# cmavro/GNN-RAG

Measured on AMD Instinct MI355X. Metric: kg_edges_aggregated_per_sec, higher is better.
Workload: dtype f32

## Files before the change

gnn-rag_amd/_lib.py:

```python
from __future__ import annotations

import ctypes as C
import os

PKG = os.path.dirname(os.path.abspath(__file__))
LIB_PATH = os.path.join(PKG, "lib", "libgnnrag_hip.so")

c_i32p = C.POINTER(C.c_int32)
c_f32p = C.POINTER(C.c_float)


class CsrStruct(C.Structure):
    _fields_ = [
        ("B", C.c_int32), ("N", C.c_int32), ("R1", C.c_int32), ("heavy_deg", C.c_int32),
        ("F", C.c_int64),
        ("row_ptr", C.c_void_p * 2), ("edge", C.c_void_p * 2), ("perm", C.c_void_p * 2),
        ("w_gnn", C.c_void_p * 2), ("w_rel", C.c_void_p * 2),
        ("heavy", C.c_void_p * 2), ("chunk_off", C.c_void_p * 2),
        ("n_heavy", C.c_void_p), ("n_chunks", C.c_void_p),
        ("heavy_cap", C.c_int32), ("max_chunks", C.c_int32),
        ("big_cnt", C.c_void_p), ("big_nodes", C.c_void_p),
        ("big_deg", C.c_int32), ("hub_sorted", C.c_int32),
        ("edge_l", C.c_void_p * 2), ("rel_off", C.c_void_p), ("rel_rows", C.c_void_p),
        ("rel_total", C.c_int32), ("rel_max", C.c_int32),
# ... 81 lines not shown
                                            C.c_int32, C.c_int32, _VP]),
    "gnnrag_update_score": (C.c_int, [_VP, _VP, _VP, _VP, _VP, _VP, _VP, _VP, _VP, C.c_int64, C.c_int32,
                                      C.c_int32, C.c_int32, _VP]),
    "gnnrag_dense_form": (C.c_int, [C.c_int32, C.c_int64, C.c_int32, C.c_int32, C.c_int32, C.c_int32, C.c_int64,
                                    C.c_int32, C.c_int32, C.POINTER(DenseFormStruct)]),
    "gnnrag_masked_softmax": (C.c_int, [_VP, _VP, C.c_int32, C.c_int32, _VP]),
    "gnnrag_typelayer": (C.c_int, [C.POINTER(CsrStruct), _VP, C.c_int, _VP, C.c_int32, _VP, C.c_size_t, _VP]),
    "gnnrag_layer_workspace_bytes": (C.c_size_t, [C.POINTER(CsrStruct), C.c_int32, C.c_int32]),
    "gnnrag_stack_workspace_bytes": (C.c_size_t, [C.POINTER(CsrStruct), C.c_int32, C.c_int32, C.c_int32]),
    "gnnrag_rel_transform": (C.c_int, [_VP, _VP, C.c_int64, C.c_int32, C.c_int32, C.POINTER(LayerParams), C.c_int32, _VP,
                                      _VP, _VP]),
    "gnnrag_gemm_tn_workspace_bytes": (C.c_size_t, [C.c_int64, C.c_int32, C.c_int32]),
    "gnnrag_gemm_tn": (C.c_int, [_VP, _VP, C.c_int64, C.c_int32, C.c_int32, _VP, _VP, C.c_size_t, _VP]),
    "gnnrag_rel_planes_bytes": (C.c_size_t, [C.c_int64, C.c_int32, C.c_int32]),
    "gnnrag_relation_tables_planes": (C.c_int, [C.POINTER(CsrStruct), _VP, _VP, _VP, _VP, C.c_int32, C.c_int32, _VP]),
    "gnnrag_reason_layer": (C.c_int, [C.POINTER(CsrStruct)] + [_VP] * 9 + [C.c_int32] + [_VP] * 8 +
                            [_VP, C.c_size_t, C.c_int32, C.c_int32, C.c_int32, C.c_int32, _VP]),
    "gnnrag_reason_stack": (C.c_int, [C.POINTER(CsrStruct), C.c_int32, C.POINTER(LayerParams)] + [_VP] * 5 +
                            [C.c_int32] + [_VP] * 6 + [_VP, C.c_size_t, C.c_int32, C.c_int32, C.c_int32, C.c_int32, _VP]),
    "gnnrag_reason_stack_capture": (C.c_int, [C.POINTER(CsrStruct), C.c_int32, C.POINTER(LayerParams)] + [_VP] * 5 +
                                    [C.c_int32] + [_VP] * 6 + [_VP, C.c_size_t, C.c_int32, C.c_int32, C.c_int32,
                                                               C.c_int32, _VP, C.POINTER(C.c_void_p)]),
    "gnnrag_graph_launch": (C.c_int, [_VP, _VP]),
    "gnnrag_graph_destroy": (C.c_int, [_VP]),
    "gnnrag_frontier_workspace_bytes": (C.c_size_t, [C.POINTER(CsrStruct)]),
    "gnnrag_frontier_supported": (C.c_int, [C.POINTER(CsrStruct), C.c_int32]),
    "gnnrag_frontier_build": (C.c_int, [C.POINTER(CsrStruct), _VP, _VP, C.c_size_t, _VP]),
    "gnnrag_relation_tables_frontier": (C.c_int, [C.POINTER(CsrStruct), _VP, _VP, _VP, _VP, _VP, _VP, C.c_int32,
                                                  C.c_int32, _VP]),
    "gnnrag_aggregate_fused_frontier": (C.c_int, [C.POINTER(CsrStruct), _VP, _VP, _VP, _VP, C.c_int32, _VP]),
# ... 99 lines not shown
```

gnn-rag_amd/csrc/dense_internal.h:

```cpp
#pragma once
#include "gnnrag_common.h"

namespace gnnrag {

int tables_vq_launch_z(const gnnrag_csr* csr, const void* planes, const float* ins, const float* W, float* P, int32_t D,
                       int32_t I, int32_t only_dir, float* zero, int64_t zero_n, hipStream_t stream);

int update_score_fused_rows(const float* h, const float* nbr, const uint8_t* add_flag, const float* W, const float* b,
                            const float* w_s, const float* b_s, const float* mask, float* h_out, float* score,
                            int64_t BN, int32_t D, int32_t I, int32_t math, hipStream_t stream, bool score_zeroed);
int update_b3_launch_f(const float* h, const float* nbr, const uint8_t* add_flag, const float* W, const float* b,
                       const float* w_s, const float* b_s, const float* mask, float* h_out, float* score, int64_t BN,
                       int32_t D, int32_t ldw, hipStream_t stream, bool score_zeroed);

bool update_rows_supported(const float* h, const float* nbr, const float* W, const float* h_out, int64_t BN, int32_t D,
                           int32_t I, int32_t math);
bool update_b3_shape_ok(int64_t BN, int32_t D, int32_t ldw);
int tables_small_launch(const gnnrag_csr* csr, const float* T_fwd, const float* T_inv, const float* ins, const float* W,
                        float* P, int32_t D, int32_t I, hipStream_t stream);

int frontier_build_z(const gnnrag_csr* csr, const float* dist, void* fws, size_t fws_bytes, float* zero_a,
                     int64_t zero_na, float* zero_b, int64_t zero_nb, hipStream_t stream);
const uint8_t* frontier_row_flags(const gnnrag_csr* csr, const void* fws);

int update_score_fused_z(const float* h, const float* nbr, const float* W, const float* b, const float* w_s,
                         const float* b_s, const float* mask, float* h_out, float* score, int64_t BN, int32_t D,
                         int32_t I, int32_t math, hipStream_t stream, bool score_zeroed);

bool rel_transform_accepts(const float* relfeat_fwd, const float* relfeat_inv, int64_t R1, int32_t D, int32_t L,
                           const gnnrag_layer_params* layers, int32_t pos_rows, const float* T_out, const void* planes_out);

}
```

gnn-rag_amd/csrc/rel_transform.hip:

```cpp
#include "gnnrag_common.h"
#include "dense_internal.h"

namespace gnnrag {

constexpr int kRtMaxL = 8;
constexpr int kRtUnroll = 7;

struct RelTArgs {
  const float* A[2];
  const float* W[kRtMaxL];
  const float* b[kRtMaxL];
  const float* add[kRtMaxL][2];
  float* C;
  unsigned short* planes;
  int M, K, N, add_rows;
};

constexpr int kPlaneHalf = 224;
constexpr int kPlaneRow = 2 * kPlaneHalf;

template <int TPW>
__global__ __launch_bounds__(256) void k_rel_transform(RelTArgs g) {
  extern __shared__ __attribute__((aligned(16))) float Wf[];
  const int tid = threadIdx.x, lane = tid & 63, wave = tid >> 6;
  const int fr = lane & 15, fg = lane >> 4;
  const int j = blockIdx.z >> 1, d = blockIdx.z & 1;
  const int colg = blockIdx.y * 64;
  const int K = g.K;
  const int nch = (K + 15) >> 4;
  const f32x4 zero4 = {0.f, 0.f, 0.f, 0.f};
  const bool compute = colg < g.N;
  if (compute) {
    const int total = 64 * nch * 4;
    for (int x = tid; x < total; x += 256) {
// ... 1 lines not shown
      f32x4 v = zero4;
      if (colg + col < g.N && 4 * kq < K) v = *reinterpret_cast<const f32x4*>(g.W[j] + (size_t)(colg + col) * K + 4 * kq);
      const int c = kq >> 2, fgq = kq & 3, a = col & 3, frq = col >> 2;
      *reinterpret_cast<f32x4*>(Wf + ((size_t)((c * 4 + a) * 64 + fgq * 16 + frq)) * 4) = v;
    }
  }
  __syncthreads();
  const int c4 = colg + 4 * fr;
  const bool in_T = c4 < g.N;
  const bool in_pad = !in_T && c4 < kPlaneHalf;
  f32x4 bias = zero4;
  if (in_T && g.b[j]) bias = *reinterpret_cast<const f32x4*>(g.b[j] + c4);
  const float* __restrict__ addp = g.add[j][d];
  float* __restrict__ cp = g.C + ((size_t)(2 * j + d) * g.M) * g.N;
  unsigned short* pp = g.planes ? g.planes + ((size_t)(2 * j + d) * 3 * g.M) * kPlaneRow : nullptr;

#pragma unroll 1
  for (int t = 0; t < TPW; ++t) {
    const int row0 = (blockIdx.x * TPW + t) * 64 + wave * 16;
    if (row0 >= g.M) break;
    f32x4 acc[4][2];
#pragma unroll
    for (int a = 0; a < 4; ++a) acc[a][0] = acc[a][1] = zero4;
    if (compute) {
      const float* __restrict__ ap = g.A[d] + (size_t)min(row0 + fr, g.M - 1) * K;
      for (int c0 = 0; c0 < nch; c0 += kRtUnroll) {
        f32x4 av[kRtUnroll];
#pragma unroll
        for (int u = 0; u < kRtUnroll; ++u)
          av[u] = *reinterpret_cast<const f32x4*>(ap + min(16 * (c0 + u) + 4 * fg, K - 4));
// ... 1 lines not shown
        for (int u = 0; u < kRtUnroll; ++u) {
          const int c = min(c0 + u, nch - 1);
          const bool live = 16 * (c0 + u) + 4 * fg < K;
          const f32x4 x = live ? av[u] : zero4;
          f32x4 wv[4];
#pragma unroll
          for (int a = 0; a < 4; ++a) wv[a] = *reinterpret_cast<const f32x4*>(Wf + ((size_t)((c * 4 + a) * 64 + lane)) * 4);
#pragma unroll
          for (int e = 0; e < 4; ++e)
#pragma unroll
            for (int a = 0; a < 4; ++a)
              acc[a][e & 1] = __builtin_amdgcn_mfma_f32_16x16x4f32(x[e], wv[a][e], acc[a][e & 1], 0, 0, 0);
        }
      }
    }
    if (!in_T && !(pp && in_pad)) continue;
#pragma unroll
    for (int r = 0; r < 4; ++r) {
      const int row = row0 + 4 * fg + r;
      if (row >= g.M) continue;
      f32x4 v = zero4;
      if (in_T) {
#pragma unroll
        for (int a = 0; a < 4; ++a) v[a] = acc[a][0][r] + acc[a][1][r];
        v += bias;
        if (addp && row < g.add_rows) v += *reinterpret_cast<const f32x4*>(addp + (size_t)row * g.N + c4);
        *reinterpret_cast<f32x4*>(cp + (size_t)row * g.N + c4) = v;
      }
      if (pp) {
#pragma unroll
        for (int half = 0; half < 2; ++half) {
          const Split3 sp = split3(__builtin_elementwise_max(half ? -v : v, zero4));
          const size_t e = (size_t)row * kPlaneRow + half * kPlaneHalf + c4;
          *reinterpret_cast<uint2*>(pp + e) = sp.hi;
          *reinterpret_cast<uint2*>(pp + (size_t)g.M * kPlaneRow + e) = sp.mid;
          *reinterpret_cast<uint2*>(pp + (size_t)2 * g.M * kPlaneRow + e) = sp.lo;
        }
      }
    }
  }
}

}

using namespace gnnrag;

extern "C" size_t gnnrag_rel_planes_bytes(int64_t R1, int32_t D, int32_t L) {
  if (R1 <= 0 || D <= 0 || D > kPlaneHalf || L <= 0) return 0;
  return (size_t)L * 2 * 3 * R1 * kPlaneRow * sizeof(unsigned short);
}

bool gnnrag::rel_transform_accepts(const float* relfeat_fwd, const float* relfeat_inv, int64_t R1, int32_t D, int32_t L,
                                   const gnnrag_layer_params* layers, int32_t pos_rows, const float* T_out,
                                   const void* planes_out) {
  if (D <= 0 || (D & 3)) return false;
  if (planes_out && D > kPlaneHalf) return false;
  if (R1 >= ((int64_t)1 << 31) / D) return false;
  uintptr_t align = (uintptr_t)relfeat_fwd | (uintptr_t)relfeat_inv | (uintptr_t)T_out | (uintptr_t)planes_out;
  for (int j = 0; j < L; ++j) {
    align |= (uintptr_t)layers[j].W_rel | (uintptr_t)layers[j].b_rel;
    if (pos_rows > 0) align |= (uintptr_t)layers[j].pos_fwd | (uintptr_t)layers[j].pos_inv;
  }
  if (align & 15) return false;
  return (size_t)64 * ((D + 15) / 16) * 16 * sizeof(float) <= 160 * 1024;
}

extern "C" int gnnrag_rel_transform(const float* relfeat_fwd, const float* relfeat_inv, int64_t R1, int32_t D,
                                    int32_t L, const gnnrag_layer_params* layers, int32_t pos_rows, float* T_out,
                                    void* planes_out, gnnrag_stream_t stream) {
  if (!relfeat_fwd || !relfeat_inv || !layers || !T_out || R1 < 0 || D <= 0 || L <= 0 || pos_rows < 0)
    return GNNRAG_E_BADARG;
  for (int j = 0; j < L; ++j) {
    if (!layers[j].W_rel) return GNNRAG_E_BADARG;
    if ((layers[j].pos_fwd == nullptr) != (layers[j].pos_inv == nullptr)) return GNNRAG_E_BADARG;
  }
  if (!gnnrag::rel_transform_accepts(relfeat_fwd, relfeat_inv, R1, D, L, layers, pos_rows, T_out, planes_out))
    return GNNRAG_E_UNSUPPORTED;
  if (R1 == 0) return 0;
  for (int j0 = 0; j0 < L; j0 += kRtMaxL) {
    const int n = L - j0 < kRtMaxL ? L - j0 : kRtMaxL;
    RelTArgs g;
    memset(&g, 0, sizeof(g));
    g.A[0] = relfeat_fwd;
    g.A[1] = relfeat_inv;
    for (int j = 0; j < n; ++j) {
      const gnnrag_layer_params& p = layers[j0 + j];
      g.W[j] = p.W_rel;
      g.b[j] = p.b_rel;
      g.add[j][0] = pos_rows > 0 ? p.pos_fwd : nullptr;
      g.add[j][1] = pos_rows > 0 ? p.pos_inv : nullptr;
    }
    g.C = T_out + (size_t)j0 * 2 * R1 * D;
    g.planes = planes_out ? (unsigned short*)planes_out + (size_t)j0 * 2 * 3 * R1 * kPlaneRow : nullptr;
    g.M = (int)R1; g.K = D; g.N = D;
    g.add_rows = (int)(pos_rows < R1 ? pos_rows : R1);
    const unsigned gy = (unsigned)(((planes_out ? kPlaneHalf : D) + 63) / 64), gz = (unsigned)(2 * n);
    const size_t lds = (size_t)64 * ((D + 15) / 16) * 16 * sizeof(float);
    static DeviceMask cap1, cap4;
    if (R1 > 2048) {
      if (lds > 64 * 1024) { const int rc = raise_lds_cap(k_rel_transform<4>, cap4); if (rc) return rc; }
      hipLaunchKernelGGL(k_rel_transform<4>, dim3((unsigned)((R1 + 255) / 256), gy, gz), dim3(256), lds,
                         (hipStream_t)stream, g);
    } else {
      if (lds > 64 * 1024) { const int rc = raise_lds_cap(k_rel_transform<1>, cap1); if (rc) return rc; }
      hipLaunchKernelGGL(k_rel_transform<1>, dim3((unsigned)((R1 + 63) / 64), gy, gz), dim3(256), lds,
                         (hipStream_t)stream, g);
    }
    GNNRAG_LAUNCH_CHECK();
  }
  return 0;
}
```

gnn-rag_amd/csrc/softmax_layer.hip:

```cpp
#include "gnnrag_common.h"
#include "dense_internal.h"

namespace gnnrag {

template <int ITEMS>
__global__ __launch_bounds__(1024) void k_masked_softmax(const float* __restrict__ score,
                                                         float* __restrict__ dist, int N) {
  __shared__ float red[16];
  __shared__ float bcast;
  const float* s = score + (size_t)blockIdx.x * N;
  float* o = dist + (size_t)blockIdx.x * N;
  const int lane = threadIdx.x & 63, wave = threadIdx.x >> 6;
  float v[ITEMS > 0 ? ITEMS : 1];

  float m = -INFINITY;
  if constexpr (ITEMS > 0) {
#pragma unroll
    for (int k = 0; k < ITEMS; ++k) {
      const int i = threadIdx.x + k * 1024;
      v[k] = i < N ? s[i] : -INFINITY;
      m = fmaxf(m, v[k]);
    }
  } else {
    for (int i = threadIdx.x; i < N; i += 1024) m = fmaxf(m, s[i]);
// ... 256 lines not shown
      if (!gated) GNNRAG_HIP(hipMemsetAsync(nbr, 0, (size_t)BN * D * sizeof(float), (hipStream_t)stream));
      rc = frontier_build_z(csr, dist, fws, w.fws_bytes, score_out, BN, nbr + (size_t)BN * D, D, (hipStream_t)stream);
      if (rc) return rc;
      rc = gnnrag_relation_tables_frontier(csr, fws, T_fwd, T_inv, ins, W_e2e, P, D, I, stream);
      if (rc) return rc;
      rc = gnnrag_aggregate_fused_frontier(csr, fws, dist, P, nbr, D, stream);
      if (rc) return rc;
      rc = update_score_fused_rows(h, nbr, gated ? frontier_row_flags(csr, fws) : nullptr, W_e2e, b_e2e, w_score, b_score,
                                   mask, h_out, score_out, BN, D, I, math, (hipStream_t)stream, true);
      if (rc) return rc;
      return finish_softmax(csr, w, base, score_out, dist_out, D, only < 0, pairs_for_next, stream);
    }
    rc = GNNRAG_E_UNSUPPORTED;
    bool score_zeroed = false;
    if (planes && math != GNNRAG_MATH_FP32 && csr->rel_total > 0) {
      rc = tables_vq_launch_z(csr, planes, ins, W_e2e, P, D, I, one_dir ? only : -1, score_out, BN, (hipStream_t)stream);
      score_zeroed = rc == 0;
    }
    if (rc == GNNRAG_E_UNSUPPORTED) rc = gnnrag_relation_tables(csr, T_fwd, T_inv, ins, W_e2e, P, D, I, math, stream);
    if (rc) return rc;
    rc = aggregate_fused_dirs(csr, dist, P, nbr, D, one_dir ? 2 - only : 0, base + w.partial, w.partial_bytes,
                              (hipStream_t)stream, pairs_ready && !one_dir);
    if (rc) return rc;
    rc = update_score_fused_z(h, nbr, W_e2e, b_e2e, w_score, b_score, mask, h_out, score_out, BN, D, I, math,
                              (hipStream_t)stream, score_zeroed);
    if (rc) return rc;
    return finish_softmax(csr, w, base, score_out, dist_out, D, only < 0, pairs_for_next, stream);
  } else {
    float* agg = (float*)(base + w.agg);
    rc = gnnrag_aggregate(csr, dist, ins, T_fwd, T_inv, agg, D, I, base + w.partial, w.partial_bytes, stream);
    if (rc) return rc;
    rc = gnnrag_update_score(h, agg, W_e2e, b_e2e, w_score, b_score, mask, h_out, score_out, BN, D, I, math,
                             stream);
    if (rc) return rc;
  }
  return gnnrag_masked_softmax(score_out, dist_out, csr->B, csr->N, stream);
}

static int rel_projections(const gnnrag_csr* csr, int32_t n, const gnnrag_layer_params* layers,
                           const float* relfeat_fwd, const float* relfeat_inv, int32_t pos_rows, float* T,
                           void* planes, bool* planes_written, int32_t D, int32_t math, gnnrag_stream_t stream) {
  *planes_written = false;
  if ((D & 3) == 0) {
    const int rc = gnnrag_rel_transform(relfeat_fwd, relfeat_inv, csr->R1, D, n, layers, pos_rows, T, planes, stream);
    if (rc == 0) *planes_written = planes != nullptr;
    if (rc != GNNRAG_E_UNSUPPORTED) return rc;
  }
  const size_t RD = (size_t)csr->R1 * D;
  for (int j = 0; j < n; ++j) {
    const gnnrag_layer_params& p = layers[j];
    const int rc = gnnrag_linear_pair(relfeat_fwd, relfeat_inv, csr->R1, D, p.W_rel, p.b_rel, p.pos_fwd, p.pos_inv,
                                      p.pos_fwd ? pos_rows : 0, T + 2 * j * RD, T + (2 * j + 1) * RD, D, math, stream);
    if (rc) return rc;
  }
  return 0;
}

extern "C" size_t gnnrag_stack_workspace_bytes(const gnnrag_csr* csr, int32_t L, int32_t D, int32_t I) {
  if (!csr || L <= 0 || D <= 0 || I <= 0) return 0;
// ... 38 lines not shown
  if (!csr || L <= 0 || !layers || !h0 || !dist0 || !ins || !relfeat_fwd || !relfeat_inv || !w_score || !b_score ||
      !mask || !h_out || !score_out || !dist_out || !workspace || D <= 0 || I <= 0)
    return GNNRAG_E_BADARG;
  if (!path_ok(path)) return GNNRAG_E_BADARG;
  for (int j = 0; j < L; ++j)
    if (!layers[j].W_rel || !layers[j].b_rel || !layers[j].W_e2e || !layers[j].b_e2e) return GNNRAG_E_BADARG;
  const LayerWs w = layer_ws(csr, D, I);
  if (workspace_bytes < w.total) return GNNRAG_E_WORKSPACE;
  char* base = (char*)workspace;
  const size_t BN = (size_t)csr->B * csr->N;
  const size_t RD = (size_t)csr->R1 * D;
  const bool upfront = L > 1 && workspace_bytes >= gnnrag_stack_workspace_bytes(csr, L, D, I);
  float* T0 = (float*)(base + w.T_fwd);
  float* Tall = (float*)(base + w.total);
  const bool want_planes = planes_wanted(csr, D, I, path, math);
  const size_t plane_bytes = tables_vq_planes_bytes(csr->R1);
  char* planes_all = base + w.total + align_up((size_t)L * 2 * RD * sizeof(float), 256);
  bool planes_written = false;
  const bool reuse = upfront && (path & GNNRAG_PATH_REUSE_PROJ) != 0;
  path &= ~GNNRAG_PATH_REUSE_PROJ;
  if (reuse) {
    planes_written = want_planes && rel_transform_accepts(relfeat_fwd, relfeat_inv, csr->R1, D, L, layers, pos_rows, Tall,
                                                          planes_all);
  } else if (upfront) {
    const int rc = rel_projections(csr, L, layers, relfeat_fwd, relfeat_inv, pos_rows, Tall,
                                   want_planes ? planes_all : nullptr, &planes_written, D, math, stream);
    if (rc) return rc;
  }
  const float* h = h0;
  const float* dist = dist0;
  bool pairs_ready = false;
// ... 92 lines not shown
```

gnn-rag_amd/csrc/tables_b3.hip:

```cpp
#include "gnnrag_common.h"
#include "dense_internal.h"
#include "b3_tile.h"
#include <type_traits>

namespace gnnrag {

#ifndef GNNRAG_TAB_TPW
#define GNNRAG_TAB_TPW 3
#endif
#ifndef GNNRAG_TAB_MINBLK
#define GNNRAG_TAB_MINBLK 2
#endif
constexpr int kTabTPW = GNNRAG_TAB_TPW;
constexpr int kTabQBytes = 160 * 1024 - 3 * kTabPlaneB - 64;

struct TabArgs {
  const float* T[2];
  const float* ins;
  const float* W;
  float* P;
  const int2* rows;
  int32_t M, D, I, ldw;
  int32_t ct0;
  int32_t npass;
// ... 258 lines not shown
#pragma unroll
  for (int pl = 0; pl < 3; ++pl) {
    const uint4 c = make_uint4(r.p[pl].x | r.n[pl].x, r.p[pl].y | r.n[pl].y, r.p[pl].z | r.n[pl].z, r.p[pl].w | r.n[pl].w);
    o.pl[pl] = __builtin_bit_cast(bf16x8, c);
  }
  const unsigned m[4] = {r.n[0].x | r.n[1].x | r.n[2].x, r.n[0].y | r.n[1].y | r.n[2].y, r.n[0].z | r.n[1].z | r.n[2].z,
                         r.n[0].w | r.n[1].w | r.n[2].w};
  unsigned ix = 0x8888u;
#pragma unroll
  for (int i = 0; i < 4; ++i)
    ix |= (min(m[i] & 0xffffu, 1u) | (min(m[i] >> 16, 1u) << 2)) << (4 * i);
  o.idx = (int)ix;
  return o;
}

template <int CTN>
__device__ __forceinline__ void tables_vq_part(const VqArgs& a, unsigned char* lds, int col0) {
  constexpr int RB = kTabRowB, PL = kTabPlaneB;
  constexpr int NPAIR = (kVqTPW + 1) / 2;
  const int tid = threadIdx.x, lane = tid & 63, wave = tid >> 6;
  const int fr = lane & 15, fg = lane >> 4;
  const int d = a.dir0 + blockIdx.y;
  const int g = blockIdx.x / a.nchunk, ch = blockIdx.x - g * a.nchunk;
  const int D = a.D, I = a.I;
  const int r0 = a.rel_off[g], r1 = a.rel_off[g + 1];
  if (r1 <= r0) return;
  const int ncol = min(CTN * 16, D - col0);
  const f32x4 zero4 = {0.f, 0.f, 0.f, 0.f};
  float* P = a.P + (size_t)d * a.M * D;
  const unsigned char* planes = a.planes + (size_t)d * 3 * a.R1 * kVqRowB;
  const size_t plane_stride = (size_t)a.R1 * kVqRowB;

  const int U = (r1 - r0 + 15) >> 4;
  const int c0 = U * ch / a.nchunk, c1 = U * (ch + 1) / a.nchunk;
  const int wv = __builtin_amdgcn_readfirstlane(wave);
  const int w0 = c0 + (c1 - c0) * wv / 8, w1 = c0 + (c1 - c0) * (wv + 1) / 8;
  const int npass = ((c1 - c0 + 7) / 8 + kVqTPW - 1) / kVqTPW;

  float* qarea = reinterpret_cast<float*>(lds + 3 * PL + 64);
  for (int x = tid * 4; x < I * D; x += 512 * 4)
    *reinterpret_cast<f32x4*>(qarea + x) = *reinterpret_cast<const f32x4*>(a.ins + (size_t)g * I * D + x);

  for (int pass = 0; pass < npass; ++pass) {
    const int tbase = w0 + pass * kVqTPW;
    const int ntile = max(0, min(kVqTPW, w1 - tbase));
    f32x4 acc[kVqTPW][CTN];
#pragma unroll
    for (int j = 0; j < kVqTPW; ++j)
#pragma unroll
      for (int nt = 0; nt < CTN; ++nt) acc[j][nt] = zero4;
    unsigned aoff[kVqTPW];
#pragma unroll
    for (int j = 0; j < kVqTPW; ++j) {
      const int m = min(r0 + (tbase + (j < ntile ? j : 0)) * 16 + fr, r1 - 1);
      aoff[j] = (unsigned)a.rows[m].y * (unsigned)kVqRowB + (unsigned)fg * 16u;
    }
    const unsigned char* const plane_base[3] = {planes, planes + plane_stride, planes + 2 * plane_stride};

    for (int s = 0; s < 3; ++s) {
      __syncthreads();
      const int nblk = s < 2 ? 3 : 1;
      vq_stage<CTN, GNNRAG_VQ_UN>(a, lds, qarea, col0, ncol, d, 3 * s, nblk);
      __syncthreads();
      for (int kb = 0; kb < nblk; ++kb) {
        const int blk = 3 * s + kb;
        const unsigned char* wb = lds + fr * RB + kb * 64 + fg * 16;
#pragma unroll
        for (int p = 0; p < NPAIR; ++p) {
          const int j0 = 2 * p, j1 = 2 * p + 1 < kVqTPW ? 2 * p + 1 : 2 * p;
          const bool two = 2 * p + 1 < kVqTPW;
          VqA cur[2];
          {
            cur[0] = vq_compress(vq_load_a(plane_base, aoff[j0] + (unsigned)(blk * 64)));
            cur[1] = two ? vq_compress(vq_load_a(plane_base, aoff[j1] + (unsigned)(blk * 64))) : cur[0];
          }
          auto products = [&](auto two_c) {
#pragma unroll
            for (int nt = 0; nt < CTN; ++nt) {
              bf16x16 b[3];
#pragma unroll
              for (int pl = 0; pl < 3; ++pl) b[pl] = vq_read_b(wb + pl * PL + nt * 16 * RB);
#pragma unroll
              for (int q = 0; q < 6; ++q) {
                acc[j0][nt] = __builtin_amdgcn_smfmac_f32_16x16x64_bf16(cur[0].pl[kB3PA[q]], b[kB3PB[q]], acc[j0][nt], cur[0].idx, 0, 0);
                if (decltype(two_c)::value)
                  acc[j1][nt] = __builtin_amdgcn_smfmac_f32_16x16x64_bf16(cur[1].pl[kB3PA[q]], b[kB3PB[q]], acc[j1][nt], cur[1].idx, 0, 0);
              }
            }
          };
          if (two && j0 < ntile) products(std::true_type{});
          else if (!two && j0 < ntile) products(std::false_type{});
        }
      }
    }

#pragma unroll
    for (int j = 0; j < kVqTPW; ++j)
      if (j < ntile) tab_store_tiles<CTN>(acc[j], P, D, r0 + (tbase + j) * 16, r1, col0, ncol, fr, fg);
  }
}

__global__ __launch_bounds__(512, 2) void k_tables_vq(VqArgs a) {
  extern __shared__ __attribute__((aligned(16))) unsigned char lds[];
  if (a.zero) {
    const int64_t nb = (int64_t)gridDim.x * gridDim.y * gridDim.z;
    const int64_t lin = blockIdx.x + (int64_t)gridDim.x * (blockIdx.y + (int64_t)gridDim.y * blockIdx.z);
    for (int64_t i = lin * 512 + threadIdx.x; i < a.zero_n; i += nb * 512) a.zero[i] = 0.f;
  }
  const int NT = (a.D + 15) >> 4;
  const int h = blockIdx.z;
  const int ctn = h == 0 ? a.ct0 : NT - a.ct0;
  const int col0 = h == 0 ? 0 : a.ct0 * 16;
  switch (ctn) {
    case 6: tables_vq_part<6>(a, lds, col0); break;
    case 7: tables_vq_part<7>(a, lds, col0); break;
    default: break;
  }
}

struct UpdB3Args {
  const float* A;
  const float* W;
  const float* bias;
  const float* add;
  const float* w_s;
  const float* b_s;
  const float* mask;
  float* C;
  float* score;
  const uint8_t* add_flag;
// ... 203 lines not shown
  const int chunks = b3_row_chunks(cus / 2, (BN + 15) / 16);
  if (!score_zeroed) GNNRAG_HIP(hipMemsetAsync(score, 0, (size_t)BN * sizeof(float), stream));
  static DeviceMask cap, cap_f;
  {
    const int rc = add_flag ? raise_lds_cap(k_update_b3<true>, cap_f) : raise_lds_cap(k_update_b3<false>, cap);
    if (rc) return rc;
  }
  const int nblk = ((chunks + 7) / 8) * 16;
  if (add_flag) hipLaunchKernelGGL(k_update_b3<true>, dim3(nblk), dim3(512), 160 * 1024, stream, a, chunks);
  else hipLaunchKernelGGL(k_update_b3<false>, dim3(nblk), dim3(512), 160 * 1024, stream, a, chunks);
  GNNRAG_LAUNCH_CHECK();
  return 0;
}

size_t tables_vq_planes_bytes(int64_t R1) { return (size_t)2 * 3 * R1 * kVqRowB; }

bool tables_vq_shape_ok(int32_t D, int32_t I) {
  return b3_shape_ok(D) && I >= 1 && (size_t)I * D * sizeof(float) <= (size_t)kTabQBytes;
}

int tables_vq_launch(const gnnrag_csr* csr, const void* planes, const float* ins, const float* W, float* P, int32_t D,
                     int32_t I, int32_t only_dir, hipStream_t stream) {
  return tables_vq_launch_z(csr, planes, ins, W, P, D, I, only_dir, nullptr, 0, stream);
}

int tables_vq_launch_z(const gnnrag_csr* csr, const void* planes, const float* ins, const float* W, float* P, int32_t D,
                       int32_t I, int32_t only_dir, float* zero, int64_t zero_n, hipStream_t stream) {
  if (!tables_vq_shape_ok(D, I) || csr->rel_total < 1024 || only_dir > 1) return GNNRAG_E_UNSUPPORTED;
  if (!aligned16(planes, ins, W, P)) return GNNRAG_E_UNSUPPORTED;
  VqArgs a;
  memset(&a, 0, sizeof(a));
  a.planes = (const unsigned char*)planes; a.ins = ins; a.W = W; a.P = P;
  a.rows = (const int2*)csr->rel_rows; a.rel_off = csr->rel_off;
  a.M = csr->rel_total; a.D = D; a.I = I; a.ldw = (2 * I + 1) * D; a.R1 = csr->R1;
  const int NT = (D + 15) / 16;
  a.ct0 = (NT + 1) / 2;
  int cus = 0;
  {
    const int rc = device_cu_count(&cus);
    if (rc) return rc;
  }
  const int ndir = only_dir < 0 ? 2 : 1;
  a.dir0 = only_dir < 0 ? 0 : only_dir;
  int nchunk = cus / (csr->B * 2 * ndir);
  const int tiles_max = (csr->rel_max + 15) / 16;
  if (nchunk > tiles_max / 8) nchunk = tiles_max / 8;
  if (nchunk < 1) nchunk = 1;
  a.nchunk = nchunk;
  a.zero = zero;
  a.zero_n = zero ? zero_n : 0;
  static DeviceMask cap;
  {
    const int rc = raise_lds_cap(k_tables_vq, cap);
    if (rc) return rc;
  }
  hipLaunchKernelGGL(k_tables_vq, dim3(csr->B * nchunk, ndir, 2), dim3(512), 160 * 1024, stream, a);
  GNNRAG_LAUNCH_CHECK();
  return 0;
}

int tables_b3_launch(const gnnrag_csr* csr, const float* T_fwd, const float* T_inv, const float* ins, const float* W,
                     float* P, int32_t D, int32_t I, hipStream_t stream) {
  if (!b3_shape_ok(D) || csr->rel_total < 1024) return GNNRAG_E_UNSUPPORTED;
  if (!aligned16(T_fwd, T_inv, ins, W, P)) return GNNRAG_E_UNSUPPORTED;
  TabArgs a;
  memset(&a, 0, sizeof(a));
  a.T[0] = T_fwd; a.T[1] = T_inv; a.ins = ins; a.W = W; a.P = P;
  a.rows = (const int2*)csr->rel_rows;
  a.M = csr->rel_total; a.D = D; a.I = I; a.ldw = (2 * I + 1) * D;
  const int NT = (D + 15) / 16;
  a.ct0 = NT <= kTabNTH ? NT : (NT + 1) / 2;
// ... 14 lines not shown
    if (rc) return rc;
  }
  hipLaunchKernelGGL(k_tables_b3, dim3(chunks, 2, parts), dim3(512), lds, stream, a);
  GNNRAG_LAUNCH_CHECK();
  return 0;
}

}

extern "C" int gnnrag_relation_tables_planes(const gnnrag_csr* csr, const void* planes, const float* ins, const float* W,
                                             float* P, int32_t D, int32_t I, gnnrag_stream_t stream) {
  if (!csr || !planes || !ins || !W || !P || D <= 0 || I <= 0 || csr->rel_total < 0) return GNNRAG_E_BADARG;
  if (csr->rel_total == 0) return 0;
  return gnnrag::tables_vq_launch(csr, planes, ins, W, P, D, I, -1, (hipStream_t)stream);
}
```

gnn-rag_amd/ops.py:

```python
from __future__ import annotations

import collections
import ctypes as C
import os
from typing import Optional

import numpy as np
import torch

from . import _lib


MATH_FP32, MATH_BF16X3, MATH_MIXED = 0, 1, 2
MATH_NAMES = {MATH_FP32: "fp32 (v_mfma_f32_16x16x4_f32, bit-exact fmaf chains)",
              MATH_BF16X3: "bf16x3 (exact 3-way bf16 split, 6 plane products on v_mfma_f32_16x16x32_bf16, fp32 accumulate)",
              MATH_MIXED: "mixed (per kernel the faster fp32-class form: bf16x3 - exact 3-way bf16 split, 6 plane products, "
                          "fp32 accumulate - for the relation tables and the self-block update, exact fp32 MFMA for the "
                          "small products)"}
_default_math = {"fp32": MATH_FP32, "bf16x3": MATH_BF16X3, "mixed": MATH_MIXED}[os.environ.get("GNNRAG_MATH", "mixed")]


def set_dense_math(mode: int) -> int:
    global _default_math
    if mode not in (MATH_FP32, MATH_BF16X3, MATH_MIXED):
# ... 311 lines not shown
        raise ValueError("W is %s, A is %s" % (tuple(W.shape), tuple(A.shape)))
    bias = None if bias is None else _chk(bias, "bias", shape=(Nout,))
    add_rows = 0
    if add is not None:
        add = _chk(add, "add")
        if add.shape[1] != Nout:
            raise ValueError("add must have %d columns" % Nout)
        add_rows = add.shape[0]
    out = _buf((M, Nout), torch.float32, A.device, "linear: out")
    with torch.cuda.device(A.device):
        _lib.check(lib.gnnrag_linear(A.data_ptr(), M, K, W.data_ptr(), _ptr(bias), _ptr(add), add_rows,
                                     int(relu), out.data_ptr(), Nout, _math(math), _stream()), "gnnrag_linear")
    return out


def rel_transform(relfeat: torch.Tensor, relfeat_inv: torch.Tensor, layers, planes: bool = False):
    lib = _lib.load()
    relfeat = _chk(relfeat, "rel_features")
    R1, D = relfeat.shape
    relfeat_inv = _chk(relfeat_inv, "rel_features_inv", shape=(R1, D))
    L = len(layers)
    params = (_lib.LayerParams * max(L, 1))()
    keep, pos_rows = [], 0
    for j, (W, b, pos, pos_inv) in enumerate(layers):
        W = _chk(W, "rel_linear.weight", shape=(D, D))
        b = _chk(b, "rel_linear.bias", shape=(D,))
        keep += [W, b]
        params[j].W_rel, params[j].b_rel = W.data_ptr(), b.data_ptr()
        if pos is not None:
            pos = _chk(pos, "pos_emb.weight")
            pos_inv = _chk(pos_inv, "pos_emb_inv.weight", shape=tuple(pos.shape))
            if pos.shape[1] != D or (pos_rows and pos.shape[0] != pos_rows):
                raise ValueError("pos_emb must be [rows, D], the same size in every layer")
            pos_rows = pos.shape[0]
            keep += [pos, pos_inv]
            params[j].pos_fwd, params[j].pos_inv = pos.data_ptr(), pos_inv.data_ptr()
    out = _buf((L, 2, R1, D), torch.float32, relfeat.device, "rel_transform: out")
    pl = None
    if planes:
        nbytes = lib.gnnrag_rel_planes_bytes(R1, D, L)
        if nbytes == 0:
            raise _lib.GnnragError("relation planes need a hidden size <= 224")
        pl = _buf((L, 2, 3, R1, nbytes // (L * 6 * R1 * 2)), torch.int16, relfeat.device, "rel_transform: planes")
    with torch.cuda.device(relfeat.device):
        _lib.check(lib.gnnrag_rel_transform(relfeat.data_ptr(), relfeat_inv.data_ptr(), R1, D, L, params, pos_rows,
                                            out.data_ptr(), _ptr(pl), _stream()), "gnnrag_rel_transform")
    return (out, pl) if planes else out


def relation_tables_planes(plan: "CsrPlan", planes: torch.Tensor, ins: torch.Tensor, W_e2e: torch.Tensor) -> torch.Tensor:
    lib = _lib.load()
    ins = _chk(ins, "relational_ins")
    B, I, D = ins.shape
    if (planes.dtype != torch.int16 or tuple(planes.shape[:3]) != (2, 3, plan.R1) or not planes.is_contiguous()
            or B != plan.B):
        raise ValueError("planes must be a contiguous [2, 3, R1, 448] int16 tensor of this plan's relation count")
    W_e2e = _chk(W_e2e, "e2e_linear.weight", shape=(D, (2 * I + 1) * D))
    _on_plan_device(plan, ins, "relational_ins")
    P = _buf((2, max(plan.rel_total, 1), D), torch.float32, ins.device, "relation_tables_planes: P")
    with torch.cuda.device(ins.device):
        _lib.check(lib.gnnrag_relation_tables_planes(C.byref(plan.c), planes.data_ptr(), ins.data_ptr(), W_e2e.data_ptr(),
                                                     P.data_ptr(), D, I, _stream()), "gnnrag_relation_tables_planes")
    return P[:, :plan.rel_total]


def gemm_tn(A: torch.Tensor, B: torch.Tensor) -> torch.Tensor:
    lib = _lib.load()
    A = _chk(A, "A")
    B = _chk(B, "B")
    if A.dim() != 2 or B.dim() != 2 or A.shape[0] != B.shape[0]:
        raise ValueError("A is %s, B is %s" % (tuple(A.shape), tuple(B.shape)))
    M, N1 = A.shape
    N2 = B.shape[1]
    out = _buf((N1, N2), torch.float32, A.device, "gemm_tn: C")
    with torch.cuda.device(A.device):
        ws = _buf(max(lib.gnnrag_gemm_tn_workspace_bytes(M, N1, N2), 16), torch.uint8, A.device, "gemm_tn: workspace")
        _lib.check(lib.gnnrag_gemm_tn(A.data_ptr(), B.data_ptr(), M, N1, N2, out.data_ptr(), ws.data_ptr(), ws.numel(),
# ... 1353 lines not shown
```

include/gnnrag.h:

```cpp
#ifndef GNNRAG_H_
#define GNNRAG_H_

#include <stddef.h>
#include <stdint.h>

#ifdef __cplusplus
extern "C" {
#endif

#define GNNRAG_ABI_VERSION 16

#define GNNRAG_E_BADARG      (-1)
#define GNNRAG_E_UNSUPPORTED (-2)
#define GNNRAG_E_WORKSPACE   (-3)
#define GNNRAG_E_TUPLE       (-4)

typedef void* gnnrag_stream_t;

typedef struct gnnrag_csr {
  int32_t B;
  int32_t N;
  int32_t R1;
  int32_t heavy_deg;
  int64_t F;
// ... 193 lines not shown
  const float* pos_fwd;
  const float* pos_inv;
  const float* W_e2e;
  const float* b_e2e;
} gnnrag_layer_params;
size_t gnnrag_stack_workspace_bytes(const gnnrag_csr* csr, int32_t L, int32_t D, int32_t I);

size_t gnnrag_rel_planes_bytes(int64_t R1, int32_t D, int32_t L);
int gnnrag_rel_transform(const float* relfeat_fwd, const float* relfeat_inv, int64_t R1, int32_t D, int32_t L,
                         const gnnrag_layer_params* layers, int32_t pos_rows, float* T_out, void* planes_out,
                         gnnrag_stream_t stream);

int gnnrag_relation_tables_planes(const gnnrag_csr* csr, const void* planes, const float* ins, const float* W,
                                  float* P, int32_t D, int32_t I, gnnrag_stream_t stream);

int gnnrag_reason_stack(const gnnrag_csr* csr, int32_t L, const gnnrag_layer_params* layers,
                        const float* h0, const float* dist0, const float* ins,
                        const float* relfeat_fwd, const float* relfeat_inv, int32_t pos_rows,
                        const float* w_score, const float* b_score, const float* mask,
                        float* h_out, float* score_out, float* dist_out,
                        void* workspace, size_t workspace_bytes,
                        int32_t D, int32_t I, int32_t path, int32_t math, gnnrag_stream_t stream);

typedef struct gnnrag_graph gnnrag_graph;
int gnnrag_reason_stack_capture(const gnnrag_csr* csr, int32_t L, const gnnrag_layer_params* layers,
                                const float* h0, const float* dist0, const float* ins,
                                const float* relfeat_fwd, const float* relfeat_inv, int32_t pos_rows,
                                const float* w_score, const float* b_score, const float* mask,
                                float* h_out, float* score_out, float* dist_out,
                                void* workspace, size_t workspace_bytes,
// ... 193 lines not shown
```

Baseline: 3.047 billion.

## Pack relation split-bf16 planes with precomputed sign index at transform time

The relation transform now writes a packed per-row operand: three bf16 magnitude planes of the absolute value plus a precomputed sign/index byte table, interleaved in one row. The tables kernel reads this operand directly instead of loading three separate plane arrays and compressing them on the fly. This is meant to cut global reads and per-tile compress arithmetic in the hot relation-table kernel, at the cost of a little extra work in the transform kernel and a new layout that both kernels must agree on. The reason-stack path switches to the packed form by default.

Result: faster. 3.204 billion (median of 6 runs) (+5.1%).

```diff
diff --git a/gnn-rag_amd/_lib.py b/gnn-rag_amd/_lib.py
--- a/gnn-rag_amd/_lib.py
+++ b/gnn-rag_amd/_lib.py
@@ -119,6 +119,11 @@
     "gnnrag_gemm_tn": (C.c_int, [_VP, _VP, C.c_int64, C.c_int32, C.c_int32, _VP, _VP, C.c_size_t, _VP]),
     "gnnrag_rel_planes_bytes": (C.c_size_t, [C.c_int64, C.c_int32, C.c_int32]),
     "gnnrag_relation_tables_planes": (C.c_int, [C.POINTER(CsrStruct), _VP, _VP, _VP, _VP, C.c_int32, C.c_int32, _VP]),
+    "gnnrag_rel_packed_bytes": (C.c_size_t, [C.c_int64, C.c_int32, C.c_int32]),
+    "gnnrag_rel_transform_packed": (C.c_int, [_VP, _VP, C.c_int64, C.c_int32, C.c_int32, C.POINTER(LayerParams), C.c_int32,
+                                             _VP, _VP, _VP]),
+    "gnnrag_relation_tables_packed": (C.c_int, [C.POINTER(CsrStruct), _VP, _VP, _VP, _VP, C.c_int32, C.c_int32, C.c_int32,
+                                               _VP]),
     "gnnrag_reason_layer": (C.c_int, [C.POINTER(CsrStruct)] + [_VP] * 9 + [C.c_int32] + [_VP] * 8 +
                             [_VP, C.c_size_t, C.c_int32, C.c_int32, C.c_int32, C.c_int32, _VP]),
     "gnnrag_reason_stack": (C.c_int, [C.POINTER(CsrStruct), C.c_int32, C.POINTER(LayerParams)] + [_VP] * 5 +
diff --git a/gnn-rag_amd/csrc/dense_internal.h b/gnn-rag_amd/csrc/dense_internal.h
--- a/gnn-rag_amd/csrc/dense_internal.h
+++ b/gnn-rag_amd/csrc/dense_internal.h
@@ -4,7 +4,8 @@
 namespace gnnrag {
 
 int tables_vq_launch_z(const gnnrag_csr* csr, const void* planes, const float* ins, const float* W, float* P, int32_t D,
-                       int32_t I, int32_t only_dir, float* zero, int64_t zero_n, hipStream_t stream);
+                       int32_t I, int32_t only_dir, float* zero, int64_t zero_n, hipStream_t stream, bool packed);
+size_t tables_vq_packed_bytes(int64_t R1);
 
 int update_score_fused_rows(const float* h, const float* nbr, const uint8_t* add_flag, const float* W, const float* b,
                             const float* w_s, const float* b_s, const float* mask, float* h_out, float* score,
@@ -29,5 +30,8 @@
 
 bool rel_transform_accepts(const float* relfeat_fwd, const float* relfeat_inv, int64_t R1, int32_t D, int32_t L,
                            const gnnrag_layer_params* layers, int32_t pos_rows, const float* T_out, const void* planes_out);
+int rel_transform_launch(const float* relfeat_fwd, const float* relfeat_inv, int64_t R1, int32_t D, int32_t L,
+                         const gnnrag_layer_params* layers, int32_t pos_rows, float* T_out, void* planes_out,
+                         void* packed_out, gnnrag_stream_t stream);
 
 }
diff --git a/gnn-rag_amd/csrc/rel_transform.hip b/gnn-rag_amd/csrc/rel_transform.hip
--- a/gnn-rag_amd/csrc/rel_transform.hip
+++ b/gnn-rag_amd/csrc/rel_transform.hip
@@ -13,11 +13,15 @@
   const float* add[kRtMaxL][2];
   float* C;
   unsigned short* planes;
+  unsigned char* packed;
   int M, K, N, add_rows;
 };
 
 constexpr int kPlaneHalf = 224;
 constexpr int kPlaneRow = 2 * kPlaneHalf;
+constexpr int kPackPlaneB = kPlaneHalf * 2;
+constexpr int kPackIdxB = 3 * kPackPlaneB;
+constexpr int kPackRowB = kPackIdxB + 64;
 
 template <int TPW>
 __global__ __launch_bounds__(256) void k_rel_transform(RelTArgs g) {
@@ -49,6 +53,7 @@
   const float* __restrict__ addp = g.add[j][d];
   float* __restrict__ cp = g.C + ((size_t)(2 * j + d) * g.M) * g.N;
   unsigned short* pp = g.planes ? g.planes + ((size_t)(2 * j + d) * 3 * g.M) * kPlaneRow : nullptr;
+  unsigned char* pk = g.packed ? g.packed + ((size_t)(2 * j + d) * g.M) * kPackRowB : nullptr;
 
 #pragma unroll 1
   for (int t = 0; t < TPW; ++t) {
@@ -80,7 +85,7 @@
         }
       }
     }
-    if (!in_T && !(pp && in_pad)) continue;
+    if (!in_T && !(pp && in_pad) && !pk) continue;
 #pragma unroll
     for (int r = 0; r < 4; ++r) {
       const int row = row0 + 4 * fg + r;
@@ -102,6 +107,19 @@
           *reinterpret_cast<uint2*>(pp + (size_t)g.M * kPlaneRow + e) = sp.mid;
           *reinterpret_cast<uint2*>(pp + (size_t)2 * g.M * kPlaneRow + e) = sp.lo;
         }
+      }
+      if (pk) {
+        unsigned char* rowp = pk + (size_t)row * kPackRowB;
+        if (c4 < kPlaneHalf) {
+          const Split3 sp = split3(__builtin_elementwise_abs(v));
+          *reinterpret_cast<uint2*>(rowp + 2 * c4) = sp.hi;
+          *reinterpret_cast<uint2*>(rowp + kPackPlaneB + 2 * c4) = sp.mid;
+          *reinterpret_cast<uint2*>(rowp + 2 * kPackPlaneB + 2 * c4) = sp.lo;
+        }
+        const int q = c4 >> 2;
+        const unsigned ix = 0x88u | (unsigned)(v[0] < 0.f) | (unsigned)(v[1] < 0.f) << 2 | (unsigned)(v[2] < 0.f) << 4 |
+                            (unsigned)(v[3] < 0.f) << 6;
+        rowp[kPackIdxB + ((q & 7) >> 1) * 16 + (q >> 3) * 2 + (q & 1)] = (unsigned char)(c4 < kPlaneHalf ? ix : 0u);
       }
     }
   }
@@ -131,16 +149,23 @@
   return (size_t)64 * ((D + 15) / 16) * 16 * sizeof(float) <= 160 * 1024;
 }
 
-extern "C" int gnnrag_rel_transform(const float* relfeat_fwd, const float* relfeat_inv, int64_t R1, int32_t D,
-                                    int32_t L, const gnnrag_layer_params* layers, int32_t pos_rows, float* T_out,
-                                    void* planes_out, gnnrag_stream_t stream) {
+extern "C" size_t gnnrag_rel_packed_bytes(int64_t R1, int32_t D, int32_t L) {
+  if (R1 <= 0 || D <= 0 || D > kPlaneHalf || L <= 0) return 0;
+  return (size_t)L * 2 * R1 * kPackRowB;
+}
+
+int gnnrag::rel_transform_launch(const float* relfeat_fwd, const float* relfeat_inv, int64_t R1, int32_t D, int32_t L,
+                                 const gnnrag_layer_params* layers, int32_t pos_rows, float* T_out, void* planes_out,
+                                 void* packed_out, gnnrag_stream_t stream) {
+  if (planes_out && packed_out) return GNNRAG_E_BADARG;
+  void* const side_out = planes_out ? planes_out : packed_out;
   if (!relfeat_fwd || !relfeat_inv || !layers || !T_out || R1 < 0 || D <= 0 || L <= 0 || pos_rows < 0)
     return GNNRAG_E_BADARG;
   for (int j = 0; j < L; ++j) {
     if (!layers[j].W_rel) return GNNRAG_E_BADARG;
     if ((layers[j].pos_fwd == nullptr) != (layers[j].pos_inv == nullptr)) return GNNRAG_E_BADARG;
   }
-  if (!gnnrag::rel_transform_accepts(relfeat_fwd, relfeat_inv, R1, D, L, layers, pos_rows, T_out, planes_out))
+  if (!gnnrag::rel_transform_accepts(relfeat_fwd, relfeat_inv, R1, D, L, layers, pos_rows, T_out, side_out))
     return GNNRAG_E_UNSUPPORTED;
   if (R1 == 0) return 0;
   for (int j0 = 0; j0 < L; j0 += kRtMaxL) {
@@ -158,9 +183,10 @@
     }
     g.C = T_out + (size_t)j0 * 2 * R1 * D;
     g.planes = planes_out ? (unsigned short*)planes_out + (size_t)j0 * 2 * 3 * R1 * kPlaneRow : nullptr;
+    g.packed = packed_out ? (unsigned char*)packed_out + (size_t)j0 * 2 * R1 * kPackRowB : nullptr;
     g.M = (int)R1; g.K = D; g.N = D;
     g.add_rows = (int)(pos_rows < R1 ? pos_rows : R1);
-    const unsigned gy = (unsigned)(((planes_out ? kPlaneHalf : D) + 63) / 64), gz = (unsigned)(2 * n);
+    const unsigned gy = (unsigned)(((side_out ? kPlaneHalf : D) + 63) / 64), gz = (unsigned)(2 * n);
     const size_t lds = (size_t)64 * ((D + 15) / 16) * 16 * sizeof(float);
     static DeviceMask cap1, cap4;
     if (R1 > 2048) {
@@ -176,3 +202,16 @@
   }
   return 0;
 }
+
+extern "C" int gnnrag_rel_transform(const float* relfeat_fwd, const float* relfeat_inv, int64_t R1, int32_t D,
+                                    int32_t L, const gnnrag_layer_params* layers, int32_t pos_rows, float* T_out,
+                                    void* planes_out, gnnrag_stream_t stream) {
+  return gnnrag::rel_transform_launch(relfeat_fwd, relfeat_inv, R1, D, L, layers, pos_rows, T_out, planes_out, nullptr, stream);
+}
+
+extern "C" int gnnrag_rel_transform_packed(const float* relfeat_fwd, const float* relfeat_inv, int64_t R1, int32_t D,
+                                           int32_t L, const gnnrag_layer_params* layers, int32_t pos_rows, float* T_out,
+                                           void* packed_out, gnnrag_stream_t stream) {
+  if (!packed_out) return GNNRAG_E_BADARG;
+  return gnnrag::rel_transform_launch(relfeat_fwd, relfeat_inv, R1, D, L, layers, pos_rows, T_out, nullptr, packed_out, stream);
+}
diff --git a/gnn-rag_amd/csrc/softmax_layer.hip b/gnn-rag_amd/csrc/softmax_layer.hip
--- a/gnn-rag_amd/csrc/softmax_layer.hip
+++ b/gnn-rag_amd/csrc/softmax_layer.hip
@@ -294,7 +294,7 @@
     rc = GNNRAG_E_UNSUPPORTED;
     bool score_zeroed = false;
     if (planes && math != GNNRAG_MATH_FP32 && csr->rel_total > 0) {
-      rc = tables_vq_launch_z(csr, planes, ins, W_e2e, P, D, I, one_dir ? only : -1, score_out, BN, (hipStream_t)stream);
+      rc = tables_vq_launch_z(csr, planes, ins, W_e2e, P, D, I, one_dir ? only : -1, score_out, BN, (hipStream_t)stream, true);
       score_zeroed = rc == 0;
     }
     if (rc == GNNRAG_E_UNSUPPORTED) rc = gnnrag_relation_tables(csr, T_fwd, T_inv, ins, W_e2e, P, D, I, math, stream);
@@ -322,7 +322,7 @@
                            void* planes, bool* planes_written, int32_t D, int32_t math, gnnrag_stream_t stream) {
   *planes_written = false;
   if ((D & 3) == 0) {
-    const int rc = gnnrag_rel_transform(relfeat_fwd, relfeat_inv, csr->R1, D, n, layers, pos_rows, T, planes, stream);
+    const int rc = rel_transform_launch(relfeat_fwd, relfeat_inv, csr->R1, D, n, layers, pos_rows, T, nullptr, planes, stream);
     if (rc == 0) *planes_written = planes != nullptr;
     if (rc != GNNRAG_E_UNSUPPORTED) return rc;
   }
@@ -391,7 +391,7 @@
   float* T0 = (float*)(base + w.T_fwd);
   float* Tall = (float*)(base + w.total);
   const bool want_planes = planes_wanted(csr, D, I, path, math);
-  const size_t plane_bytes = tables_vq_planes_bytes(csr->R1);
+  const size_t plane_bytes = tables_vq_packed_bytes(csr->R1);
   char* planes_all = base + w.total + align_up((size_t)L * 2 * RD * sizeof(float), 256);
   bool planes_written = false;
   const bool reuse = upfront && (path & GNNRAG_PATH_REUSE_PROJ) != 0;
diff --git a/gnn-rag_amd/csrc/tables_b3.hip b/gnn-rag_amd/csrc/tables_b3.hip
--- a/gnn-rag_amd/csrc/tables_b3.hip
+++ b/gnn-rag_amd/csrc/tables_b3.hip
@@ -296,9 +296,22 @@
   return o;
 }
 
-template <int CTN>
+constexpr int kVqPackPlaneB = kVqHalf * 2;
+constexpr int kVqPackIdxB = 3 * kVqPackPlaneB;
+constexpr int kVqPackRowB = kVqPackIdxB + 64;
+__device__ __forceinline__ VqA vq_load_packed(const unsigned char* row_base, unsigned off, int blk) {
+  VqA o;
+#pragma unroll
+  for (int pl = 0; pl < 3; ++pl)
+    o.pl[pl] = __builtin_bit_cast(bf16x8, *reinterpret_cast<const uint4*>(row_base + (off + (unsigned)(pl * kVqPackPlaneB + blk * 64))));
+  o.idx = *reinterpret_cast<const unsigned short*>(row_base + (off + (unsigned)(kVqPackIdxB + blk * 2)));
+  return o;
+}
+
+template <int CTN, bool PACKED>
 __device__ __forceinline__ void tables_vq_part(const VqArgs& a, unsigned char* lds, int col0) {
   constexpr int RB = kTabRowB, PL = kTabPlaneB;
+  constexpr unsigned AROWB = PACKED ? kVqPackRowB : kVqRowB;
   constexpr int NPAIR = (kVqTPW + 1) / 2;
   const int tid = threadIdx.x, lane = tid & 63, wave = tid >> 6;
   const int fr = lane & 15, fg = lane >> 4;
@@ -310,7 +323,7 @@
   const int ncol = min(CTN * 16, D - col0);
   const f32x4 zero4 = {0.f, 0.f, 0.f, 0.f};
   float* P = a.P + (size_t)d * a.M * D;
-  const unsigned char* planes = a.planes + (size_t)d * 3 * a.R1 * kVqRowB;
+  const unsigned char* planes = a.planes + (size_t)d * (PACKED ? 1 : 3) * a.R1 * AROWB;
   const size_t plane_stride = (size_t)a.R1 * kVqRowB;
 
   const int U = (r1 - r0 + 15) >> 4;
@@ -335,7 +348,7 @@
 #pragma unroll
     for (int j = 0; j < kVqTPW; ++j) {
       const int m = min(r0 + (tbase + (j < ntile ? j : 0)) * 16 + fr, r1 - 1);
-      aoff[j] = (unsigned)a.rows[m].y * (unsigned)kVqRowB + (unsigned)fg * 16u;
+      aoff[j] = (unsigned)a.rows[m].y * AROWB + (unsigned)fg * 16u;
     }
     const unsigned char* const plane_base[3] = {planes, planes + plane_stride, planes + 2 * plane_stride};
 
@@ -352,7 +365,10 @@
           const int j0 = 2 * p, j1 = 2 * p + 1 < kVqTPW ? 2 * p + 1 : 2 * p;
           const bool two = 2 * p + 1 < kVqTPW;
           VqA cur[2];
-          {
+          if constexpr (PACKED) {
+            cur[0] = vq_load_packed(planes, aoff[j0], blk);
+            cur[1] = two ? vq_load_packed(planes, aoff[j1], blk) : cur[0];
+          } else {
             cur[0] = vq_compress(vq_load_a(plane_base, aoff[j0] + (unsigned)(blk * 64)));
             cur[1] = two ? vq_compress(vq_load_a(plane_base, aoff[j1] + (unsigned)(blk * 64))) : cur[0];
           }
@@ -382,6 +398,7 @@
   }
 }
 
+template <bool PACKED>
 __global__ __launch_bounds__(512, 2) void k_tables_vq(VqArgs a) {
   extern __shared__ __attribute__((aligned(16))) unsigned char lds[];
   if (a.zero) {
@@ -394,8 +411,8 @@
   const int ctn = h == 0 ? a.ct0 : NT - a.ct0;
   const int col0 = h == 0 ? 0 : a.ct0 * 16;
   switch (ctn) {
-    case 6: tables_vq_part<6>(a, lds, col0); break;
-    case 7: tables_vq_part<7>(a, lds, col0); break;
+    case 6: tables_vq_part<6, PACKED>(a, lds, col0); break;
+    case 7: tables_vq_part<7, PACKED>(a, lds, col0); break;
     default: break;
   }
 }
@@ -629,6 +646,8 @@
 }
 
 size_t tables_vq_planes_bytes(int64_t R1) { return (size_t)2 * 3 * R1 * kVqRowB; }
+size_t tables_vq_packed_bytes(int64_t R1) { return (size_t)2 * R1 * kVqPackRowB; }
+static_assert(2 * kVqPackRowB <= 2 * 3 * kVqRowB, "a layer's packed operand fits the slot of its planes");
 
 bool tables_vq_shape_ok(int32_t D, int32_t I) {
   return b3_shape_ok(D) && I >= 1 && (size_t)I * D * sizeof(float) <= (size_t)kTabQBytes;
@@ -636,12 +655,13 @@
 
 int tables_vq_launch(const gnnrag_csr* csr, const void* planes, const float* ins, const float* W, float* P, int32_t D,
                      int32_t I, int32_t only_dir, hipStream_t stream) {
-  return tables_vq_launch_z(csr, planes, ins, W, P, D, I, only_dir, nullptr, 0, stream);
+  return tables_vq_launch_z(csr, planes, ins, W, P, D, I, only_dir, nullptr, 0, stream, false);
 }
 
 int tables_vq_launch_z(const gnnrag_csr* csr, const void* planes, const float* ins, const float* W, float* P, int32_t D,
-                       int32_t I, int32_t only_dir, float* zero, int64_t zero_n, hipStream_t stream) {
+                       int32_t I, int32_t only_dir, float* zero, int64_t zero_n, hipStream_t stream, bool packed) {
   if (!tables_vq_shape_ok(D, I) || csr->rel_total < 1024 || only_dir > 1) return GNNRAG_E_UNSUPPORTED;
+  if ((int64_t)csr->R1 * (packed ? kVqPackRowB : kVqRowB) >= ((int64_t)1 << 32)) return GNNRAG_E_UNSUPPORTED;
   if (!aligned16(planes, ins, W, P)) return GNNRAG_E_UNSUPPORTED;
   VqArgs a;
   memset(&a, 0, sizeof(a));
@@ -664,12 +684,13 @@
   a.nchunk = nchunk;
   a.zero = zero;
   a.zero_n = zero ? zero_n : 0;
-  static DeviceMask cap;
+  static DeviceMask cap, cap_p;
   {
-    const int rc = raise_lds_cap(k_tables_vq, cap);
+    const int rc = packed ? raise_lds_cap(k_tables_vq<true>, cap_p) : raise_lds_cap(k_tables_vq<false>, cap);
     if (rc) return rc;
   }
-  hipLaunchKernelGGL(k_tables_vq, dim3(csr->B * nchunk, ndir, 2), dim3(512), 160 * 1024, stream, a);
+  if (packed) hipLaunchKernelGGL(k_tables_vq<true>, dim3(csr->B * nchunk, ndir, 2), dim3(512), 160 * 1024, stream, a);
+  else hipLaunchKernelGGL(k_tables_vq<false>, dim3(csr->B * nchunk, ndir, 2), dim3(512), 160 * 1024, stream, a);
   GNNRAG_LAUNCH_CHECK();
   return 0;
 }
@@ -714,3 +735,11 @@
   if (csr->rel_total == 0) return 0;
   return gnnrag::tables_vq_launch(csr, planes, ins, W, P, D, I, -1, (hipStream_t)stream);
 }
+
+extern "C" int gnnrag_relation_tables_packed(const gnnrag_csr* csr, const void* packed, const float* ins, const float* W,
+                                             float* P, int32_t D, int32_t I, int32_t only_dir, gnnrag_stream_t stream) {
+  if (!csr || !packed || !ins || !W || !P || D <= 0 || I <= 0 || csr->rel_total < 0 || only_dir < -1 || only_dir > 1)
+    return GNNRAG_E_BADARG;
+  if (csr->rel_total == 0) return 0;
+  return gnnrag::tables_vq_launch_z(csr, packed, ins, W, P, D, I, only_dir, nullptr, 0, (hipStream_t)stream, true);
+}
diff --git a/gnn-rag_amd/ops.py b/gnn-rag_amd/ops.py
--- a/gnn-rag_amd/ops.py
+++ b/gnn-rag_amd/ops.py
@@ -349,7 +349,9 @@
     return out
 
 
-def rel_transform(relfeat: torch.Tensor, relfeat_inv: torch.Tensor, layers, planes: bool = False):
+def rel_transform(relfeat: torch.Tensor, relfeat_inv: torch.Tensor, layers, planes: bool = False, packed: bool = False):
+    if planes and packed:
+        raise ValueError("planes and packed are two forms of the same operand: ask for one")
     lib = _lib.load()
     relfeat = _chk(relfeat, "rel_features")
     R1, D = relfeat.shape
@@ -377,10 +379,20 @@
         if nbytes == 0:
             raise _lib.GnnragError("relation planes need a hidden size <= 224")
         pl = _buf((L, 2, 3, R1, nbytes // (L * 6 * R1 * 2)), torch.int16, relfeat.device, "rel_transform: planes")
+    if packed:
+        nbytes = lib.gnnrag_rel_packed_bytes(R1, D, L)
+        if nbytes == 0:
+            raise _lib.GnnragError("the packed relation operand needs a hidden size <= 224")
+        pl = _buf((L, 2, R1, nbytes // (L * 2 * R1)), torch.uint8, relfeat.device, "rel_transform: packed")
     with torch.cuda.device(relfeat.device):
-        _lib.check(lib.gnnrag_rel_transform(relfeat.data_ptr(), relfeat_inv.data_ptr(), R1, D, L, params, pos_rows,
-                                            out.data_ptr(), _ptr(pl), _stream()), "gnnrag_rel_transform")
-    return (out, pl) if planes else out
+        if packed:
+            _lib.check(lib.gnnrag_rel_transform_packed(relfeat.data_ptr(), relfeat_inv.data_ptr(), R1, D, L, params,
+                                                       pos_rows, out.data_ptr(), _ptr(pl), _stream()),
+                       "gnnrag_rel_transform_packed")
+        else:
+            _lib.check(lib.gnnrag_rel_transform(relfeat.data_ptr(), relfeat_inv.data_ptr(), R1, D, L, params, pos_rows,
+                                                out.data_ptr(), _ptr(pl), _stream()), "gnnrag_rel_transform")
+    return (out, pl) if planes or packed else out
 
 
 def relation_tables_planes(plan: "CsrPlan", planes: torch.Tensor, ins: torch.Tensor, W_e2e: torch.Tensor) -> torch.Tensor:
@@ -396,6 +408,27 @@
     with torch.cuda.device(ins.device):
         _lib.check(lib.gnnrag_relation_tables_planes(C.byref(plan.c), planes.data_ptr(), ins.data_ptr(), W_e2e.data_ptr(),
                                                      P.data_ptr(), D, I, _stream()), "gnnrag_relation_tables_planes")
+    return P[:, :plan.rel_total]
+
+
+def relation_tables_packed(plan: "CsrPlan", packed: torch.Tensor, ins: torch.Tensor, W_e2e: torch.Tensor,
+                           only_dir: int = -1) -> torch.Tensor:
+    lib = _lib.load()
+    ins = _chk(ins, "relational_ins")
+    B, I, D = ins.shape
+    if (packed.dtype != torch.uint8 or packed.dim() != 3 or tuple(packed.shape[:2]) != (2, plan.R1)
+            or not packed.is_contiguous() or B != plan.B):
+        raise ValueError("packed must be a contiguous [2, R1, 1408] uint8 tensor of this plan's relation count")
+    if only_dir not in (-1, 0, 1):
+        raise ValueError("only_dir is -1, 0 or 1")
+    W_e2e = _chk(W_e2e, "e2e_linear.weight", shape=(D, (2 * I + 1) * D))
+    _on_plan_device(plan, ins, "relational_ins")
+    P = _buf((2, max(plan.rel_total, 1), D), torch.float32, ins.device, "relation_tables_packed: P")
+    if only_dir >= 0:
+        P.zero_()
+    with torch.cuda.device(ins.device):
+        _lib.check(lib.gnnrag_relation_tables_packed(C.byref(plan.c), packed.data_ptr(), ins.data_ptr(), W_e2e.data_ptr(),
+                                                     P.data_ptr(), D, I, only_dir, _stream()), "gnnrag_relation_tables_packed")
     return P[:, :plan.rel_total]
 
 
diff --git a/include/gnnrag.h b/include/gnnrag.h
--- a/include/gnnrag.h
+++ b/include/gnnrag.h
@@ -231,6 +231,13 @@
 int gnnrag_relation_tables_planes(const gnnrag_csr* csr, const void* planes, const float* ins, const float* W,
                                   float* P, int32_t D, int32_t I, gnnrag_stream_t stream);
 
+size_t gnnrag_rel_packed_bytes(int64_t R1, int32_t D, int32_t L);
+int gnnrag_rel_transform_packed(const float* relfeat_fwd, const float* relfeat_inv, int64_t R1, int32_t D, int32_t L,
+                                const gnnrag_layer_params* layers, int32_t pos_rows, float* T_out, void* packed_out,
+                                gnnrag_stream_t stream);
+int gnnrag_relation_tables_packed(const gnnrag_csr* csr, const void* packed, const float* ins, const float* W,
+                                  float* P, int32_t D, int32_t I, int32_t only_dir, gnnrag_stream_t stream);
+
 int gnnrag_reason_stack(const gnnrag_csr* csr, int32_t L, const gnnrag_layer_params* layers,
                         const float* h0, const float* dist0, const float* ins,
                         const float* relfeat_fwd, const float* relfeat_inv, int32_t pos_rows,
```
